# nexus1203/libBICOS

Measured on AMD Instinct MI355X. Metric: disparity Mpix/s + ms/match, 33x2 stack @ 2048x1536, 1/2/4/8 MI355X, higher is better.
Workload: dtype u8; 1 GPU; cfg2: 33x2 stack @ 2048x1536 u8, LIMITED 128-bit (4n-7=125 bits), nxcorr 0.96; n_images=33, rows=1536, cols=2048, descriptor_bits=128, rows_per_rank=1536, parallelism=single GPU

## Files before the change

### include/bicos_c.h

```cpp
#ifndef BICOS_C_H
#define BICOS_C_H

#include <stddef.h>
#include <stdint.h>

#ifdef __cplusplus
extern "C" {
#endif

#define BICOS_CV_8U 0
#define BICOS_CV_16U 2
#define BICOS_CV_16S 3
#define BICOS_CV_32F 5
#define BICOS_CV_64F 6

typedef struct {
    float nxcorr_threshold;
    float subpixel_step;
    float min_variance;
    int mode;
    int precision;
    int variant_type;
    int max_lr_diff;
    int no_dupes;
// ... 62 lines not shown
int bicos_match_host_range(bicos_engine* e, const void* const* stack0, const void* const* stack1,
                           int n, int rows, int cols, size_t step, int depth,
                           const BicosConfig* cfg, int has_nxcorr, int min_disparity,
                           int max_disparity, void* disparity, void* corrmap);


int bicos_match_host_multi(const int* devices, int ndev, const void* const* stack0,
                           const void* const* stack1, int n, int rows, int cols, size_t step,
                           int depth, const BicosConfig* cfg, int has_nxcorr, void* disparity,
                           void* corrmap);

int bicos_match_bands_device(const int* devices, int ndev, const void* const* stack0,
                             const void* const* stack1, const int* band_rows,
                             const size_t* row_pitch, const size_t* plane_pitch, int n, int cols,
                             int depth, const BicosConfig* cfg, int has_nxcorr, void* disparity,
                             void* corrmap);

size_t bicos_desc_pitch(int cols, int words);
int bicos_transform_device(const void* stack, int n, int rows, int cols, size_t row_pitch,
                           size_t plane_pitch, int depth, int mode, int words, uint32_t* desc,
                           void* stream);
int bicos_search_device(bicos_engine* e, const uint32_t* desc0, const uint32_t* desc1, int rows,
                        int cols, int words, int flags, int max_lr_diff, int16_t* out,
                        void* stream);
int bicos_search_device_range(bicos_engine* e, const uint32_t* desc0, const uint32_t* desc1,
                              int rows, int cols, int words, int flags, int max_lr_diff,
                              int min_disparity, int max_disparity, int16_t* out, void* stream);
int bicos_agree_device(const int16_t* raw, const void* stack0, const void* stack1, int n, int rows,
                       int cols, size_t row_pitch, size_t plane_pitch, int depth, float threshold,
                       int has_minvar, float minvar_scaled, float* out, float* corrmap,
                       void* stream);
int bicos_subpixel_device(const int16_t* raw, const void* stack0, const void* stack1, int n,
                          int rows, int cols, size_t row_pitch, size_t plane_pitch, int depth,
                          float threshold, float step, int has_minvar, float minvar_scaled,
                          float* out, float* corrmap, void* stream);
int bicos_agree_stage_device(const int16_t* raw, const void* stack0, const void* stack1, int n,
                             int rows, int cols, size_t row_pitch, size_t plane_pitch, int depth,
                             float threshold, float step, int has_minvar, float minvar_scaled,
                             int precision, float* out, void* corrmap, void* stream);

#define BICOS_PLAN_MATRIX_CORES 1
#define BICOS_PLAN_PACKED_KEYS 2
#define BICOS_PLAN_AGREE_IN_SEARCH 4
#define BICOS_PLAN_REVERSE_COMPACTED 8
#define BICOS_PLAN_CONSISTENCY_IN_AGREE 16
#define BICOS_PLAN_DENSE_ROWS 32
#define BICOS_PLAN_CONSISTENCY_ONE_PASS 64
int bicos_match_plan(bicos_engine* e, const void* stack0, const void* stack1, int n, int rows,
                     int cols, size_t row_pitch, size_t plane_pitch, int depth,
                     const BicosConfig* cfg, int has_nxcorr);
int bicos_search_packed(bicos_engine* e, int rows, int cols, int words, int bits, int n, int fused);
int bicos_agree_kernel(const void* stack0, const void* stack1, int n, size_t row_pitch,
                       size_t plane_pitch, int depth);

int bicos_search_agree_device(bicos_engine* e, const uint32_t* desc0, const uint32_t* desc1,
                              const void* stack0, const void* stack1, int n, int rows, int cols,
                              size_t row_pitch, size_t plane_pitch, int depth,
                              const BicosConfig* cfg, int has_nxcorr, void* disparity,
                              void* corrmap, void* stream);

#define BICOS_REPROJECT_ALLOW_NEGATIVE_Z 1
#define BICOS_REPROJECT_F32_SENTINEL 2
int bicos_reproject_device(bicos_engine* e, const void* disparity, int disp_type, int rows,
                           int cols, const double Q[16], int flags, float* xyz_map,
                           float* points, int32_t* index, size_t capacity, uint32_t* counts,
                           void* stream);
int bicos_reproject_host(bicos_engine* e, const void* disparity, int disp_type, int rows, int cols,
                         const double Q[16], int flags, float* xyz_map, float* points,
                         int32_t* index, size_t capacity, uint32_t counts[4]);
int bicos_reproject_segment(void);

#define BICOS_SPECKLE_F32_SENTINEL 1
int bicos_speckle_device(bicos_engine* e, const void* disparity, int disp_type, int rows, int cols,
                         int max_size, float max_diff, int flags, void* out, int32_t* labels,
                         uint32_t* counts, void* stream);
int bicos_speckle_host(bicos_engine* e, const void* disparity, int disp_type, int rows, int cols,
                       int max_size, float max_diff, int flags, void* out, int32_t* labels,
                       uint32_t counts[4]);
int bicos_speckle_tile(int* rows, int* cols);

int bicos_rectify_maps_device(const double K[9], const double* D, int nd, const double* R,
                              const double* P, int p_cols, int rows, int cols, float* map_x,
                              float* map_y, void* stream);
int bicos_rectify_maps_host(const double K[9], const double* D, int nd, const double* R,
                            const double* P, int p_cols, int rows, int cols, float* map_x,
                            float* map_y);
int bicos_rectify_device(bicos_engine* e, const void* src, int n, int src_rows, int src_cols,
                         size_t src_row_pitch, size_t src_plane_pitch, int depth,
                         const float* map_x, const float* map_y, size_t map_pitch, int rows,
                         int cols, void* dst, size_t dst_row_pitch, size_t dst_plane_pitch,
                         int border, uint8_t* valid, void* stream);
int bicos_rectify_host(bicos_engine* e, const void* const* src, int n, int src_rows, int src_cols,
                       size_t src_step, int depth, const float* map_x, const float* map_y,
                       size_t map_pitch, int rows, int cols, void* const* dst, size_t dst_step,
                       int border, uint8_t* valid);
int bicos_rectify_tile(int* rows, int* cols);

#define BICOS_MEDIAN_F32_SENTINEL 1
int bicos_median_device(bicos_engine* e, const void* disparity, int disp_type, int rows, int cols,
                        int ksize, int fill_min, int flags, void* out, uint32_t* counts, void* stream);
int bicos_median_host(bicos_engine* e, const void* disparity, int disp_type, int rows, int cols,
                      int ksize, int fill_min, int flags, void* out, uint32_t counts[4]);
int bicos_median_tile(int* rows, int* cols);

const char* bicos_build_info(void);

// ... 6 lines not shown
```

### libbicos_amd/_lib.py

```python
from __future__ import annotations

import ctypes
import os
import subprocess

_HERE = os.path.dirname(os.path.abspath(__file__))
LIB_PATH = os.path.join(_HERE, "libbicos_amd.so")
CSRC = os.path.join(_HERE, "csrc")

BICOS_OK = 0
BICOS_E_ARG = -1
BICOS_E_BITS = -2
BICOS_E_HIP = -3
BICOS_E_INTERNAL = -4

CV_8U, CV_16U, CV_16S, CV_32F, CV_64F = 0, 2, 3, 5, 6


class BicosConfig(ctypes.Structure):
    _fields_ = [
        ("nxcorr_threshold", ctypes.c_float),
        ("subpixel_step", ctypes.c_float),
        ("min_variance", ctypes.c_float),
        ("mode", ctypes.c_int),
        ("precision", ctypes.c_int),
        ("variant_type", ctypes.c_int),
        ("max_lr_diff", ctypes.c_int),
        ("no_dupes", ctypes.c_int),
    ]


class BicosResult(ctypes.Structure):
    _fields_ = [
        ("disparity_data", ctypes.c_void_p),
        ("disparity_rows", ctypes.c_int),
        ("disparity_cols", ctypes.c_int),
        ("disparity_type", ctypes.c_int),
        ("corrmap_data", ctypes.c_void_p),
        ("corrmap_rows", ctypes.c_int),
        ("corrmap_cols", ctypes.c_int),
        ("corrmap_type", ctypes.c_int),
    ]


EXPORTS = (
    "BICOS_CreateDefaultConfig", "BICOS_FreeConfig", "BICOS_FreeResult", "BICOS_Match",
    "BICOS_InvalidDisparityFloat", "BICOS_InvalidDisparityInt16", "bicos_last_error",
    "bicos_engine_create", "bicos_engine_default", "bicos_engine_destroy", "bicos_engine_tune", "bicos_descriptor_words", "bicos_output_type",
    "bicos_match_device", "bicos_match_device_i16", "bicos_match_host", "bicos_match_host_multi", "bicos_match_bands_device",
    "bicos_desc_pitch", "bicos_transform_device", "bicos_search_device",
    "bicos_agree_device", "bicos_subpixel_device", "bicos_agree_stage_device", "bicos_build_info",
    "bicos_match_plan", "bicos_search_agree_device", "bicos_search_packed", "bicos_agree_kernel",
    "bicos_match_device_range", "bicos_match_host_range", "bicos_search_device_range",
    "bicos_reproject_device", "bicos_reproject_host", "bicos_reproject_segment",
    "bicos_speckle_device", "bicos_speckle_host", "bicos_speckle_tile",
    "bicos_rectify_maps_device", "bicos_rectify_maps_host", "bicos_rectify_device",
    "bicos_rectify_host", "bicos_rectify_tile",
    "bicos_median_device", "bicos_median_host", "bicos_median_tile",
)

PLAN_MATRIX_CORES = 1
PLAN_PACKED_KEYS = 2
PLAN_AGREE_IN_SEARCH = 4
PLAN_REVERSE_COMPACTED = 8
PLAN_CONSISTENCY_IN_AGREE = 16
PLAN_DENSE_ROWS = 32
PLAN_CONSISTENCY_ONE_PASS = 64

REPROJECT_ALLOW_NEGATIVE_Z = 1
REPROJECT_F32_SENTINEL = 2

SPECKLE_F32_SENTINEL = 1

MEDIAN_F32_SENTINEL = 1


def build(verbose: bool = False, jobs: int = 4) -> str:
    out = subprocess.run(["make", "-C", CSRC, "-j%d" % jobs, "all"], capture_output=True,
                         text=True)
    if verbose:
        print(out.stdout, out.stderr)
    if out.returncode != 0:
        raise RuntimeError("libbicos_amd build failed:\n" + out.stdout[-4000:] + out.stderr[-4000:])
    return LIB_PATH


_lib = None


class BicosError(RuntimeError):
    pass


def lib() -> ctypes.CDLL:
    global _lib
    if _lib is not None:
        return _lib
    if not os.path.exists(LIB_PATH):
        raise ImportError("libbicos_amd.so not built at %s -- run libbicos_amd._lib.build() "
                          "(hipcc, gfx950)" % LIB_PATH)
    L = ctypes.CDLL(LIB_PATH)
    P, I, F, Z = ctypes.c_void_p, ctypes.c_int, ctypes.c_float, ctypes.c_size_t
    PI = ctypes.POINTER(ctypes.c_int)
    PP = ctypes.POINTER(ctypes.c_void_p)
    L.BICOS_CreateDefaultConfig.restype = ctypes.POINTER(BicosConfig)
# ... 4 lines not shown
    L.BICOS_FreeResult.restype = None
    L.BICOS_Match.argtypes = [PP, PI, PI, PI, I, PP, PI, PI, PI, I, ctypes.POINTER(BicosConfig)]
    L.BICOS_Match.restype = ctypes.POINTER(BicosResult)
    L.BICOS_InvalidDisparityFloat.restype = F
    L.BICOS_InvalidDisparityFloat.argtypes = []
    L.BICOS_InvalidDisparityInt16.restype = ctypes.c_int16
    L.BICOS_InvalidDisparityInt16.argtypes = []
    L.bicos_last_error.restype = ctypes.c_char_p
    L.bicos_last_error.argtypes = []
    L.bicos_engine_create.argtypes = [I, ctypes.POINTER(P)]
    L.bicos_engine_create.restype = I
    L.bicos_engine_default.argtypes = [I]
    L.bicos_engine_default.restype = P
    L.bicos_engine_destroy.argtypes = [P]
    L.bicos_engine_destroy.restype = None
    L.bicos_engine_tune.argtypes = [P, I, I, I, I]
    L.bicos_engine_tune.restype = I
    L.bicos_descriptor_words.argtypes = [I, I]
    L.bicos_descriptor_words.restype = I
    L.bicos_output_type.argtypes = [ctypes.POINTER(BicosConfig), I]
    L.bicos_output_type.restype = I
    L.bicos_match_device.argtypes = [P, P, P, I, I, I, Z, Z, I, ctypes.POINTER(BicosConfig), I,
                                     P, P, P]
    L.bicos_match_device.restype = I
    L.bicos_match_device_i16.argtypes = L.bicos_match_device.argtypes
    L.bicos_match_device_i16.restype = I
    L.bicos_match_host.argtypes = [P, PP, PP, I, I, I, Z, I, ctypes.POINTER(BicosConfig), I, P, P]
    L.bicos_match_host.restype = I
    PZ = ctypes.POINTER(ctypes.c_size_t)
    L.bicos_match_host_multi.argtypes = [PI, I, PP, PP, I, I, I, Z, I,
                                         ctypes.POINTER(BicosConfig), I, P, P]
    L.bicos_match_host_multi.restype = I
    L.bicos_match_bands_device.argtypes = [PI, I, PP, PP, PI, PZ, PZ, I, I, I,
                                           ctypes.POINTER(BicosConfig), I, P, P]
    L.bicos_match_bands_device.restype = I
    L.bicos_desc_pitch.argtypes = [I, I]
    L.bicos_desc_pitch.restype = Z
    L.bicos_transform_device.argtypes = [P, I, I, I, Z, Z, I, I, I, P, P]
    L.bicos_transform_device.restype = I
    L.bicos_search_device.argtypes = [P, P, P, I, I, I, I, I, P, P]
    L.bicos_search_device.restype = I
    L.bicos_agree_device.argtypes = [P, P, P, I, I, I, Z, Z, I, F, I, F, P, P, P]
    L.bicos_agree_device.restype = I
    L.bicos_subpixel_device.argtypes = [P, P, P, I, I, I, Z, Z, I, F, F, I, F, P, P, P]
    L.bicos_subpixel_device.restype = I
    L.bicos_agree_stage_device.argtypes = [P, P, P, I, I, I, Z, Z, I, F, F, I, F, I, P, P, P]
    L.bicos_agree_stage_device.restype = I
    L.bicos_match_plan.argtypes = [P, P, P, I, I, I, Z, Z, I, ctypes.POINTER(BicosConfig), I]
    L.bicos_match_plan.restype = I
    L.bicos_search_packed.argtypes = [P, I, I, I, I, I, I]
    L.bicos_search_packed.restype = I
    L.bicos_agree_kernel.argtypes = [P, P, I, Z, Z, I]
    L.bicos_agree_kernel.restype = I
    L.bicos_search_agree_device.argtypes = [P, P, P, P, P, I, I, I, Z, Z, I,
                                            ctypes.POINTER(BicosConfig), I, P, P, P]
    L.bicos_search_agree_device.restype = I
    L.bicos_match_device_range.argtypes = [P, P, P, I, I, I, Z, Z, I, ctypes.POINTER(BicosConfig),
                                           I, I, I, P, P, P]
    L.bicos_match_device_range.restype = I
    L.bicos_match_host_range.argtypes = [P, PP, PP, I, I, I, Z, I, ctypes.POINTER(BicosConfig), I,
                                         I, I, P, P]
    L.bicos_match_host_range.restype = I
    L.bicos_search_device_range.argtypes = [P, P, P, I, I, I, I, I, I, I, P, P]
    L.bicos_search_device_range.restype = I
    PD = ctypes.POINTER(ctypes.c_double)
    L.bicos_reproject_device.argtypes = [P, P, I, I, I, PD, I, P, P, P, Z, P, P]
    L.bicos_reproject_device.restype = I
    L.bicos_reproject_host.argtypes = [P, P, I, I, I, PD, I, P, P, P, Z, P]
    L.bicos_reproject_host.restype = I
    L.bicos_reproject_segment.argtypes = []
    L.bicos_reproject_segment.restype = I
    L.bicos_speckle_device.argtypes = [P, P, I, I, I, I, F, I, P, P, P, P]
    L.bicos_speckle_device.restype = I
    L.bicos_speckle_host.argtypes = [P, P, I, I, I, I, F, I, P, P, P]
    L.bicos_speckle_host.restype = I
    L.bicos_speckle_tile.argtypes = [PI, PI]
    L.bicos_speckle_tile.restype = I
    L.bicos_rectify_maps_device.argtypes = [PD, PD, I, PD, PD, I, I, I, P, P, P]
    L.bicos_rectify_maps_device.restype = I
    L.bicos_rectify_maps_host.argtypes = [PD, PD, I, PD, PD, I, I, I, P, P]
    L.bicos_rectify_maps_host.restype = I
    L.bicos_rectify_device.argtypes = [P, P, I, I, I, Z, Z, I, P, P, Z, I, I, P, Z, Z, I, P, P]
    L.bicos_rectify_device.restype = I
    L.bicos_rectify_host.argtypes = [P, PP, I, I, I, Z, I, P, P, Z, I, I, PP, Z, I, P]
    L.bicos_rectify_host.restype = I
    L.bicos_rectify_tile.argtypes = [PI, PI]
    L.bicos_rectify_tile.restype = I
    L.bicos_median_device.argtypes = [P, P, I, I, I, I, I, I, P, P, P]
    L.bicos_median_device.restype = I
    L.bicos_median_host.argtypes = [P, P, I, I, I, I, I, I, P, P]
    L.bicos_median_host.restype = I
    L.bicos_median_tile.argtypes = [PI, PI]
    L.bicos_median_tile.restype = I
    L.bicos_build_info.restype = ctypes.c_char_p
    L.bicos_build_info.argtypes = []
    _lib = L
    return L


def check_disparity_range(rng):
    if rng is None:
        return None
    try:
        lo, hi = rng
    except (TypeError, ValueError):
        raise ValueError("disparity_range must be None or a pair (lo, hi)") from None
# ... 96 lines not shown
```

### libbicos_amd/csrc/entries.cpp

```cpp
#include "engine.hpp"
#include "reproject.hpp"
#include "speckle.hpp"
#include "median.hpp"

#include <cmath>
#include <vector>

using namespace bicos_impl;

namespace {

int check_words(int words) {
    if (words == 1 || words == 2 || words == 4 || words == 8) return BICOS_OK;
    return fail(BICOS_E_ARG, "words must be 1, 2, 4 or 8");
}

int match_device_entry(bicos_engine* e, const void* stack0, const void* stack1, int n, int rows,
                       int cols, size_t row_pitch, size_t plane_pitch, int depth,
                       const BicosConfig* cfg, int has_nxcorr, void* disparity, void* corrmap,
                       void* stream, bool disp_i16, const DispRange* range = nullptr,
                       const uint32_t* desc0 = nullptr, const uint32_t* desc1 = nullptr) {
    if (range)
        if (int rc0 = check_range(range->min, range->max)) return rc0;
    if (!cfg) return fail(BICOS_E_ARG, "null config");
// ... 175 lines not shown
}

int bicos_match_device(bicos_engine* e, const void* stack0, const void* stack1, int n, int rows,
                       int cols, size_t row_pitch, size_t plane_pitch, int depth,
                       const BicosConfig* cfg, int has_nxcorr, void* disparity, void* corrmap,
                       void* stream) {
    return match_device_entry(e, stack0, stack1, n, rows, cols, row_pitch, plane_pitch, depth, cfg,
                              has_nxcorr, disparity, corrmap, stream, false);
}

int bicos_match_device_range(bicos_engine* e, const void* stack0, const void* stack1, int n,
                             int rows, int cols, size_t row_pitch, size_t plane_pitch, int depth,
                             const BicosConfig* cfg, int has_nxcorr, int min_disparity,
                             int max_disparity, void* disparity, void* corrmap, void* stream) {
    const DispRange range{min_disparity, max_disparity};
    return match_device_entry(e, stack0, stack1, n, rows, cols, row_pitch, plane_pitch, depth, cfg,
                              has_nxcorr, disparity, corrmap, stream, false, &range);
}

int bicos_match_device_i16(bicos_engine* e, const void* stack0, const void* stack1, int n, int rows,
                           int cols, size_t row_pitch, size_t plane_pitch, int depth,
                           const BicosConfig* cfg, int has_nxcorr, void* disparity, void* corrmap,
                           void* stream) {
    return match_device_entry(e, stack0, stack1, n, rows, cols, row_pitch, plane_pitch, depth, cfg,
                              has_nxcorr, disparity, corrmap, stream, true);
}

int bicos_match_plan(bicos_engine* e, const void* stack0, const void* stack1, int n, int rows,
                     int cols, size_t row_pitch, size_t plane_pitch, int depth,
                     const BicosConfig* cfg, int has_nxcorr) {
    if (!cfg) return fail(BICOS_E_ARG, "null config");
    if (int rc0 = check_stack_shape(n, depth, 0, 0)) return rc0;
    if (descriptor_words(n, cfg->mode ? 1 : 0) < 0) return fail(BICOS_E_BITS, "input stacks too large");
    return match_plan(e, n, rows, cols, row_pitch, plane_pitch, depth, *cfg, has_nxcorr != 0,
                      stack0, stack1).bits();
}

int bicos_search_packed(bicos_engine* e, int rows, int cols, int words, int bits, int n, int fused) {
    return search_runs_packed(e, rows, cols, words, bits, n, fused != 0) ? 1 : 0;
}

int bicos_agree_kernel(const void* stack0, const void* stack1, int n, size_t row_pitch,
                       size_t plane_pitch, int depth) {
    if (int rc0 = check_stack_shape(n, depth, 0, 0)) return rc0;
    bicos_hip::AgreeArgs aa{};
    aa.stack0 = stack0;
    aa.stack1 = stack1;
    aa.n = n;
    aa.row_pitch = row_pitch;
    aa.plane_pitch = plane_pitch;
    return bicos_hip::agree_kernel_kind(aa, depth);
}

int bicos_search_agree_device(bicos_engine* e, const uint32_t* desc0, const uint32_t* desc1,
                              const void* stack0, const void* stack1, int n, int rows, int cols,
                              size_t row_pitch, size_t plane_pitch, int depth,
                              const BicosConfig* cfg, int has_nxcorr, void* disparity,
                              void* corrmap, void* stream) {
    if (!cfg) return fail(BICOS_E_ARG, "null config");
    if (!e) return fail(BICOS_E_ARG, "null engine");
    if (rows > 0 && cols > 0 && (!desc0 || !desc1)) return fail(BICOS_E_ARG, "null descriptors");
    return match_device_entry(e, stack0, stack1, n, rows, cols, row_pitch, plane_pitch, depth, cfg,
                              has_nxcorr, disparity, corrmap, stream, false, nullptr, desc0, desc1);
}

int bicos_match_host(bicos_engine* e, const void* const* stack0, const void* const* stack1, int n,
                     int rows, int cols, size_t step, int depth, const BicosConfig* cfg,
                     int has_nxcorr, void* disparity, void* corrmap) {
    return match_host_entry(e, stack0, stack1, n, rows, cols, step, depth, cfg, has_nxcorr,
                            disparity, corrmap, nullptr);
}

int bicos_match_host_range(bicos_engine* e, const void* const* stack0, const void* const* stack1,
                           int n, int rows, int cols, size_t step, int depth,
                           const BicosConfig* cfg, int has_nxcorr, int min_disparity,
                           int max_disparity, void* disparity, void* corrmap) {
    const DispRange range{min_disparity, max_disparity};
    return match_host_entry(e, stack0, stack1, n, rows, cols, step, depth, cfg, has_nxcorr,
                            disparity, corrmap, &range);
}

int bicos_transform_device(const void* stack, int n, int rows, int cols, size_t row_pitch,
                           size_t plane_pitch, int depth, int mode, int words, uint32_t* desc,
                           void* stream) {
    if (int rc0 = check_stack_shape(n, depth, 0, 0)) return rc0;
    if (int rc0 = check_words(words)) return rc0;
    const int need = descriptor_words(n, mode ? 1 : 0);
    if (need < 0 || need > words) return fail(BICOS_E_BITS, "descriptor too narrow for n");
    uint32_t span = 0;
    if (int rc0 = stack_span(n, rows, cols, row_pitch, plane_pitch, depth, &span)) return rc0;
    bicos_hip::TransformArgs ta{stack, nullptr, desc, nullptr, n, rows, cols,
                                row_pitch, plane_pitch, bicos_desc_pitch(cols, words), 0, span};
    return check_hip(bicos_hip::launch_transform(ta, depth, mode ? 1 : 0, words, (hipStream_t)stream),
                     "transform launch");
}

int bicos_search_device(bicos_engine* e, const uint32_t* desc0, const uint32_t* desc1, int rows,
                        int cols, int words, int flags, int max_lr_diff, int16_t* out,
                        void* stream) {
    return search_entry(e, desc0, desc1, rows, cols, words, flags, max_lr_diff, nullptr, out,
                        stream);
}

int bicos_search_device_range(bicos_engine* e, const uint32_t* desc0, const uint32_t* desc1,
                              int rows, int cols, int words, int flags, int max_lr_diff,
                              int min_disparity, int max_disparity, int16_t* out, void* stream) {
// ... 221 lines not shown
```

### libbicos_amd/csrc/kernels.hip

```cpp
#include "kernels.hpp"
#include "nxc.hpp"
#include "stack.hpp"
#include "transform.hpp"

#include <hip/hip_runtime.h>
#include <stdint.h>

#include <algorithm>
#include <cstdlib>
#include <cstring>

#include <type_traits>

namespace bicos_hip {

namespace {

constexpr int16_t INVALID_I16 = -32768;

__device__ __forceinline__ float fdiv_rn(float a, float b) { return __fdiv_rn(a, b); }

__device__ __forceinline__ uint32_t bcnt_acc(uint32_t x, uint32_t acc) {
    asm("" : "+v"(acc));
    return __builtin_popcount(x) + acc;
}


using nxc::ld;
using nxc::fma_p;
using nxc::div_p;
using nxc::sqrt_p;
using nxc::nxcorr_dev;



template <int WORDS>
struct BitWriter {
    uint32_t w[WORDS];
    uint32_t cur = 0;
    int nbits = 0;
    int widx = 0;

    __device__ __forceinline__ BitWriter() {
#pragma unroll
        for (int k = 0; k < WORDS; ++k) w[k] = 0;
    }
    __device__ __forceinline__ void flush() {
#pragma unroll
        for (int k = 0; k < WORDS; ++k)
            if (k == widx) w[k] = cur;
    }
    __device__ __forceinline__ void set(bool v) {
        cur |= (uint32_t)v << nbits;
        if (++nbits == 32) {
            flush();
            ++widx;
// ... 55 lines not shown
                bw.set((float)a0 < av);
                ps[t] = a0 + b0;
                a0 = b0;
                b0 = c0;
            }
        }
#pragma unroll
        for (int t = 0; t < 15; ++t)
            if (t == n - 2) ps[t] = a0 + b0;
        bw.set(a0 < b0);
        bw.set((float)a0 < av);
        bw.set((float)b0 < av);
#pragma unroll
        for (int t = 0; t < 15; ++t)
#pragma unroll
            for (int i = 0; i < 15; ++i)
                if (t < n - 1 && i < n - 1 && i != t && i != t - 1 && i != t + 1)
                    bw.set(ps[t] < ps[i]);
    }
    bw.finish();

    if (WORDS % 4 == 0) {
#pragma unroll
        for (int k = 0; k < WORDS; k += 4)
            *(uint4*)(out + k) = make_uint4(bw.w[k], bw.w[k + 1], bw.w[k + 2], bw.w[k + 3]);
    } else if (WORDS == 2) {
        *(uint2*)out = make_uint2(bw.w[0], bw.w[1 % WORDS]);
    } else {
        out[0] = bw.w[0];
    }
}

template <typename TIn, int WORDS, int MAXN, bool EXACT>
__global__ __launch_bounds__(256) void transform_limited_kernel(TransformArgs a) {
    const int col = blockIdx.x * 256 + threadIdx.x;
    const int row = blockIdx.y;
    const int which = blockIdx.z;
    if (col >= a.cols) return;
    const StackReader<TIn> rd(which ? a.stack1 : a.stack0, a.stack_bytes);
    uint32_t* __restrict__ out = (which ? a.desc1 : a.desc0) + (size_t)row * a.desc_pitch + (size_t)col * WORDS;
    const uint32_t pp = (uint32_t)a.plane_pitch;
    const uint32_t rowoff = (uint32_t)row * (uint32_t)a.row_pitch;
    uint32_t w[WORDS];
    limited_descriptor<TIn, WORDS, MAXN, EXACT>(rd, (uint32_t)col, rowoff, pp, a.n, a.magic, w);

    if (WORDS % 4 == 0) {
#pragma unroll
        for (int k = 0; k < WORDS; k += 4)
            *(uint4*)(out + k) = make_uint4(w[k], w[k + 1], w[k + 2], w[k + 3]);
    } else if (WORDS == 2) {
        *(uint2*)out = make_uint2(w[0], w[1 % WORDS]);
    } else {
        out[0] = w[0];
    }
}

template <typename TIn, int WORDS, int N>
__global__ __launch_bounds__(256) void transform_full_kernel(TransformArgs a) {
    const int col = blockIdx.x * 256 + threadIdx.x;
    const int row = blockIdx.y;
    const int which = blockIdx.z;
    if (col >= a.cols) return;
    const StackReader<TIn> rd(which ? a.stack1 : a.stack0, a.stack_bytes);
    uint32_t* __restrict__ out = (which ? a.desc1 : a.desc0) + (size_t)row * a.desc_pitch + (size_t)col * WORDS;
    uint32_t w[WORDS];
    full_descriptor<TIn, WORDS, N>(rd, (uint32_t)col, (uint32_t)row * (uint32_t)a.row_pitch,
                                   (uint32_t)a.plane_pitch, a.magic, w);
    if (WORDS % 4 == 0) {
#pragma unroll
        for (int k = 0; k < WORDS; k += 4)
            *(uint4*)(out + k) = make_uint4(w[k], w[k + 1], w[k + 2], w[k + 3]);
    } else if (WORDS == 2) {
        *(uint2*)out = make_uint2(w[0], w[1 % WORDS]);
    } else {
        out[0] = w[0];
    }
}


template <int WORDS>
__device__ __forceinline__ uint32_t ham(const uint32_t (&a)[WORDS], const uint32_t (&b)[WORDS]) {
    uint32_t c = __builtin_popcount(a[0] ^ b[0]);
#pragma unroll
    for (int k = 1; k < WORDS; ++k) c = bcnt_acc(a[k] ^ b[k], c);
    return c;
}

template <int WORDS>
__device__ __forceinline__ void lds_fetch(const uint32_t* s, uint32_t (&d)[WORDS]) {
    if (WORDS >= 4) {
#pragma unroll
        for (int k = 0; k < WORDS; k += 4) {
            const uint4 v = *(const uint4*)(s + k);
            d[k] = v.x;
            d[(k + 1) % WORDS] = v.y;
            d[(k + 2) % WORDS] = v.z;
            d[(k + 3) % WORDS] = v.w;
        }
    } else if (WORDS == 2) {
        const uint2 v = *(const uint2*)s;
        d[0] = v.x;
        d[1 % WORDS] = v.y;
    } else {
        d[0] = s[0];
    }
}
// ... 307 lines not shown
    uint32_t r[MAXN];
#pragma unroll
    for (int t = 0; t < MAXN; ++t)
        r[t] = rd1(c1, rowoff + (uint32_t)min(t, n - 1) * pp);
#pragma unroll
    for (int j = 0; j < PASSES; ++j) {
        const int p = j * WPP + p0;
        if (p < n) tile_l[p * DW + threadIdx.x % DW] = w[j];
    }
    __syncthreads();
    if (!live) return;
    const TIn* lt = (const TIn*)tile_l + threadIdx.x;
    const size_t o = (size_t)row * a.cols + col;
    TPrec corr = (TPrec)__builtin_nan("");
    if (inb) {
        uint32_t sl = 0, sr = 0;
#pragma unroll
        for (int t = 0; t < MAXN; ++t)
            if (t < n) {
                sl += lt[t * 256];
                sr += r[t];
                if ((t & 7) == 7) __builtin_amdgcn_sched_barrier(0);
            }
        asm volatile("" ::: "memory");
        const TPrec m0 = div_p((TPrec)sl, (TPrec)n);
        const TPrec m1 = div_p((TPrec)sr, (TPrec)n);
        TPrec cov = 0, v0 = 0, v1 = 0;
#pragma unroll
        for (int t = 0; t < MAXN; ++t)
            if (t < n) {
                const TPrec x0 = (TPrec)(uint32_t)lt[t * 256] - m0;
                const TPrec x1 = (TPrec)r[t] - m1;
                cov = fma_p(x0, x1, cov);
                v0 = fma_p(x0, x0, v0);
                v1 = fma_p(x1, x1, v1);
                if ((t & 7) == 7) __builtin_amdgcn_sched_barrier(0);
            }
        if (a.has_minvar && (v0 < (TPrec)a.minvar || v1 < (TPrec)a.minvar))
            corr = (TPrec)-1;
        else
            corr = div_p(cov, sqrt_p(v0 * v1));
        if (corr < (TPrec)a.threshold) d = INVALID_I16;
    } else {
        d = INVALID_I16;
    }
    if (a.out_f32)
        ((float*)a.out)[o] = (float)d;
    else
        ((int16_t*)a.out)[o] = (int16_t)d;
    if (a.corrmap) ((TPrec*)a.corrmap)[o] = corr;
}


template <typename TIn, int WORDS, int MAXN>
hipError_t launch_tl(const TransformArgs& a, dim3 grid, hipStream_t st) {
    if (a.n == MAXN)
        hipLaunchKernelGGL((transform_limited_kernel<TIn, WORDS, MAXN, true>), grid, dim3(256), 0, st, a);
    else
        hipLaunchKernelGGL((transform_limited_kernel<TIn, WORDS, MAXN, false>), grid, dim3(256), 0, st, a);
    return hipGetLastError();
}

template <typename TIn, int WORDS>
hipError_t launch_transform_w(const TransformArgs& a, int mode, hipStream_t st) {
    dim3 grid((a.cols + 255) / 256, a.rows, a.stack1 ? 2 : 1);
    if (mode == 0) {
        const int n = a.n;
        if constexpr (WORDS == 1) return launch_tl<TIn, WORDS, 9>(a, grid, st);
        else if constexpr (WORDS == 2) return n <= 12 ? launch_tl<TIn, WORDS, 12>(a, grid, st)
                                                      : launch_tl<TIn, WORDS, 17>(a, grid, st);
        else if constexpr (WORDS == 4) return n <= 24 ? launch_tl<TIn, WORDS, 24>(a, grid, st)
                                                      : launch_tl<TIn, WORDS, 33>(a, grid, st);
        else if (n <= 40) return launch_tl<TIn, WORDS, 40>(a, grid, st);
        else if (n <= 48) return launch_tl<TIn, WORDS, 48>(a, grid, st);
        else return launch_tl<TIn, WORDS, 65>(a, grid, st);
    }
#define BICOS_FULL_N(N)                                                                   \
    case N:                                                                               \
        if constexpr (WORDS == (N * N - 2 * N + 3 <= 32 ? 1 : N * N - 2 * N + 3 <= 64 ? 2  \
                                : N * N - 2 * N + 3 <= 128 ? 4 : 8)) {                     \
            hipLaunchKernelGGL((transform_full_kernel<TIn, WORDS, N>), grid, dim3(256), 0, st, a); \
            return hipGetLastError();                                                     \
        }                                                                                 \
        break;
    switch (a.n) {
        BICOS_FULL_N(2) BICOS_FULL_N(3) BICOS_FULL_N(4) BICOS_FULL_N(5) BICOS_FULL_N(6)
        BICOS_FULL_N(7) BICOS_FULL_N(8) BICOS_FULL_N(9) BICOS_FULL_N(10) BICOS_FULL_N(11)
        BICOS_FULL_N(12) BICOS_FULL_N(13) BICOS_FULL_N(14) BICOS_FULL_N(15) BICOS_FULL_N(16)
    }
#undef BICOS_FULL_N
    hipLaunchKernelGGL((transform_kernel<TIn, WORDS, 1>), grid, dim3(256), 0, st, a);
    return hipGetLastError();
}

template <typename TIn>
hipError_t launch_transform_t(const TransformArgs& a, int mode, int words, hipStream_t st) {
    switch (words) {
        case 1: return launch_transform_w<TIn, 1>(a, mode, st);
        case 2: return launch_transform_w<TIn, 2>(a, mode, st);
        case 4: return launch_transform_w<TIn, 4>(a, mode, st);
        case 8: return launch_transform_w<TIn, 8>(a, mode, st);
    }
    return hipErrorInvalidValue;
}

template <int WORDS, bool NODUPES, int RP>
hipError_t launch_search16_r(const SearchArgs& a, int waves, hipStream_t st) {
    const size_t stage = (size_t)a.chunk * WORDS * 4;
// ... 80 lines not shown
    g.variant = 16;
    const int max_chunk = max_lds_bytes / (words * 4 + extra_col_bytes);
    g.chunk = cols < max_chunk ? cols : max_chunk;
    g.waves = waves ? waves : 8;
    g.R = R == 4 ? 4 : 2;
    if (split) {
        g.split = split;
    } else {
        const long base = (long)rows * ((cols + 64L * g.R - 1) / (64L * g.R));
        const int tiles256 = (cols + 255) / 256;
        const double slots = (double)(cus > 0 ? cus : 256) * 32.0;
        double best = -1.0;
        g.split = 1;
        for (int sp = 1; sp <= 8; sp *= 2) {
            if (sp > 1 && (tiles256 < sp || g.waves % sp)) break;
            const double rounds = (double)(base * sp) / slots;
            const double fill = rounds / __builtin_ceil(rounds);
            const double score = fill + 0.1 * (rounds < 3.0 ? rounds : 3.0) / 3.0 -
                                 0.005 * (double)__builtin_ctz(sp);
            if (score > best + 1e-9) {
                best = score;
                g.split = sp;
            }
        }
    }
    const long per_wg = 64L * (g.waves / g.split) * g.R;
    g.tiles_per_row = (int)((cols + per_wg - 1) / per_wg);
    return g;
}

hipError_t launch_search(SearchArgs a, const SearchGeometry& g, int words, bool nodupes,
                         hipStream_t st) {
    if (a.rows <= 0 || a.cols <= 0) return hipSuccess;
    a.chunk = g.chunk;
    a.tiles_per_row = g.tiles_per_row;
    a.split = g.split;
    if (g.waves % g.split) return hipErrorInvalidValue;
    switch (words) {
        case 1: return launch_search_w<1>(a, nodupes, g, st);
        case 2: return launch_search_w<2>(a, nodupes, g, st);
        case 4: return launch_search_w<4>(a, nodupes, g, st);
        case 8: return launch_search_w<8>(a, nodupes, g, st);
    }
    return hipErrorInvalidValue;
}

hipError_t launch_consistency(const ConsistencyArgs& a, hipStream_t st) {
    if (a.rows <= 0 || a.cols <= 0) return hipSuccess;
    dim3 grid((a.cols + 255) / 256, a.rows);
    hipLaunchKernelGGL(consistency_kernel, grid, dim3(256), 0, st, a);
    return hipGetLastError();
}

int agree_kernel_kind(const AgreeArgs& a, int depth) {
    if (a.n > 65) return 0;
    return agree_dwords_aligned(a, depth == 1 ? 1 : 2) ? 2 : 1;
}

hipError_t launch_agree(const AgreeArgs& a, int depth, bool dbl, hipStream_t st) {
    if (a.rows <= 0 || a.cols <= 0) return hipSuccess;
    if (depth == 1)
        return dbl ? launch_agree_t<uint8_t, double>(a, st) : launch_agree_t<uint8_t, float>(a, st);
    return dbl ? launch_agree_t<uint16_t, double>(a, st) : launch_agree_t<uint16_t, float>(a, st);
}

}
```

### libbicos_amd/csrc/kernels.hpp

```cpp
#pragma once

#include <hip/hip_runtime.h>
#include <stddef.h>
#include <stdint.h>

namespace bicos_hip {

struct TransformArgs {
    const void* stack0;
    const void* stack1;
    uint32_t* desc0;
    uint32_t* desc1;
    int n, rows, cols;
    size_t row_pitch;
    size_t plane_pitch;
    size_t desc_pitch;
    uint32_t magic;
    uint32_t stack_bytes;
};

struct AgreeArgs {
    const int16_t* raw;
    size_t raw_pitch;
    const void* stack0;
// ... 13 lines not shown
    const int16_t* rev;
    int max_lr_diff;
};

struct SearchArgs {
    const uint32_t* desc0;
    const uint32_t* desc1;
    int16_t* out;
    int rows, cols;
    size_t desc_pitch;
    size_t out_pitch;
    int out_mode;
    int chunk;
    int tiles_per_row;
    int split;
    int tail_col0;
    int tail_T;
    const int16_t* keep;
    size_t keep_pitch;
    uint8_t* row_valid;
    size_t valid_pitch;
};

struct SearchAgreeArgs {
    SearchArgs s;
    AgreeArgs ag;
};

struct SearchRangeArgs {
    SearchArgs s;
    int dmin, dmax;
};

struct SearchGeometry {
    int chunk;
    int waves;
    int R;
    int tiles_per_row;
    int variant;
    int split;
};

struct ConsistencyArgs {
    const int16_t* fwd;
    const int16_t* rev;
    int16_t* out;
    int rows, cols;
    size_t out_pitch;
    int max_lr_diff;
};


hipError_t launch_transform(TransformArgs a, int depth, int mode, int words, hipStream_t st);
SearchGeometry search_geometry(int rows, int cols, int words, int max_lds_bytes, int variant = 16,
                               int R = 0, int waves = 0, int split = 0, int cus = 256,
                               int extra_col_bytes = 0);
hipError_t launch_search(SearchArgs a, const SearchGeometry& g, int words, bool nodupes,
                         hipStream_t st);
hipError_t launch_consistency(const ConsistencyArgs& a, hipStream_t st);

struct MxGeometry {
    int chunk;
    int waves;
    int T;
    int tiles_per_row;
    int keys;
    int ksteps;
    int fk;
    int tail_T;
    int tail_col0;
    int pk;
    int pk_T;
    int pk_chunk;
    int pk_tiles_per_row;
    int pk_tail_col0;
    int stream;
    int prune;
    int packed;
};
MxGeometry search_mx_geometry(int rows, int cols, int words, int lds_bytes, int T = 0,
                              int waves = 0, int cus = 256, int keys = 0, int bits = 0);
hipError_t launch_search_mx(SearchArgs a, const MxGeometry& g, int words, bool nodupes,
                            hipStream_t st);
bool search_mx_agree_fusable(const MxGeometry& g, int words, bool nodupes, int cols, int n,
                             int depth, bool dbl);
hipError_t launch_search_mx_agree(SearchArgs a, const AgreeArgs& ag, const MxGeometry& g, int words,
                                  hipStream_t st);
bool search_mx_packed(const MxGeometry& g, int rows, int cols, int words, int n);
bool search_lr_eligible(int words, int bits, int cols);
hipError_t launch_search_lr(SearchArgs a, int words, int bits, int max_lr_diff, hipStream_t st);
hipError_t launch_search_range(SearchArgs a, int dmin, int dmax, int words, bool nodupes,
                               int bits, int cus, hipStream_t st, int tiles = 0,
                               int waves_wg = 0);
hipError_t launch_agree(const AgreeArgs& a, int depth, bool dbl, hipStream_t st);
int agree_kernel_kind(const AgreeArgs& a, int depth);
hipError_t launch_subpixel(const AgreeArgs& a, int depth, bool dbl, hipStream_t st);
hipError_t launch_subpixel_wide(const AgreeArgs& a, int depth, bool dbl, hipStream_t st);

}
```

### libbicos_amd/device.py

```python
from __future__ import annotations

import ctypes
import dataclasses
from typing import Optional, Sequence, Tuple

import torch

from . import _lib

INVALID_I16 = -32768


@dataclasses.dataclass
class MatchConfig:
    nxcorr_threshold: Optional[float] = 0.5
    subpixel_step: Optional[float] = None
    min_variance: Optional[float] = None
    mode: int = 0
    precision: int = 0
    variant: int = 0
    max_lr_diff: int = 1
    no_dupes: bool = False
    disparity_range: Optional[Tuple[int, int]] = None

# ... 98 lines not shown
        corr_dtype = torch.float64 if cfg.precision else torch.float32
        i16 = (out is not None and has_nxcorr and out.dtype == torch.int16 and
               cfg.subpixel_step is None)
        if i16:
            disp_dtype = torch.int16
        if out is None:
            out = torch.empty((rows, cols), dtype=disp_dtype, device=dev)
        _check_out(out, "out", (rows, cols), (disp_dtype,), dev)
        if has_nxcorr and want_corrmap and corrmap is None:
            corrmap = torch.empty((rows, cols), device=dev, dtype=corr_dtype)
        if not (has_nxcorr and want_corrmap):
            corrmap = None
        if corrmap is not None:
            _check_out(corrmap, "corrmap", (rows, cols), (corr_dtype,), dev)
        rng = _lib.check_disparity_range(cfg.disparity_range)
        if rng is not None and i16:
            raise ValueError("disparity_range is not supported with an int16 `out` map")
        if rng is not None:
            rc = self._L.bicos_match_device_range(
                self._h, stack0.data_ptr(), stack1.data_ptr(), n, rows, cols, rp, pp,
                _depth(stack0), ctypes.byref(c), has_nxcorr, rng[0], rng[1], out.data_ptr(),
                corrmap.data_ptr() if corrmap is not None else None, _stream(dev, stream))
            _lib.check(rc, "bicos_match_device_range")
            return out, corrmap
        entry = self._L.bicos_match_device_i16 if i16 else self._L.bicos_match_device
        rc = entry(
            self._h, stack0.data_ptr(), stack1.data_ptr(), n, rows, cols, rp, pp, _depth(stack0),
            ctypes.byref(c), has_nxcorr, out.data_ptr(),
            corrmap.data_ptr() if corrmap is not None else None, _stream(dev, stream))
        _lib.check(rc, "bicos_match_device")
        return out, corrmap

    def plan(self, stack0: torch.Tensor, stack1: torch.Tensor,
             cfg: Optional[MatchConfig] = None) -> int:
        cfg = cfg or MatchConfig()
        n, rows, cols, rp, pp = _check_stack(stack0)
        c, has_nxcorr = cfg.to_c()
        rc = self._L.bicos_match_plan(self._h, stack0.data_ptr(), stack1.data_ptr(), n, rows, cols,
                                      rp, pp, _depth(stack0), ctypes.byref(c), has_nxcorr)
        if rc < 0:
            _lib.check(rc, "bicos_match_plan")
        return rc

    def search_packed(self, rows: int, cols: int, words: int = 4, bits: int = 0, n: int = 0,
                      fused: bool = False) -> bool:
        return bool(self._L.bicos_search_packed(self._h, rows, cols, words, bits, n, int(fused)))

    def agree_kernel(self, stack0: torch.Tensor, stack1: torch.Tensor) -> int:
        n, rows, cols, rp, pp = _check_stack(stack0)
        rc = self._L.bicos_agree_kernel(stack0.data_ptr(), stack1.data_ptr(), n, rp, pp,
                                        _depth(stack0))
        if rc < 0:
            _lib.check(rc, "bicos_agree_kernel")
        return rc

    def search_agree(self, desc0: torch.Tensor, desc1: torch.Tensor, stack0: torch.Tensor,
                     stack1: torch.Tensor, cfg: Optional[MatchConfig] = None,
                     out: Optional[torch.Tensor] = None, corrmap: Optional[torch.Tensor] = None,
                     stream=None) -> Tuple[torch.Tensor, Optional[torch.Tensor]]:
        cfg = cfg or MatchConfig()
        n, rows, cols, rp, pp = _check_stack(stack0)
        if tuple(stack1.shape) != (n, rows, cols) or stack1.stride() != stack0.stride() or \
                stack1.dtype != stack0.dtype:
            raise ValueError("stack1 must match stack0 in shape, strides and dtype")
        words = descriptor_words(n, cfg.mode)
        pitch = self._L.bicos_desc_pitch(cols, words)
        for name, d in (("desc0", desc0), ("desc1", desc1)):
            if d.device != stack0.device or d.dtype != torch.int32 or not d.is_contiguous() or \
                    tuple(d.shape) != (rows, pitch):
                raise ValueError("%s must be a contiguous int32 [%d, %d] tensor on %s"
                                 % (name, rows, pitch, stack0.device))
        c, has_nxcorr = cfg.to_c()
        dev = stack0.device
        disp_dtype = torch.float32 if has_nxcorr else torch.int16
        corr_dtype = torch.float64 if cfg.precision else torch.float32
        if out is None:
            out = torch.empty((rows, cols), dtype=disp_dtype, device=dev)
        _check_out(out, "out", (rows, cols), (disp_dtype,), dev)
        if has_nxcorr and corrmap is None:
            corrmap = torch.empty((rows, cols), device=dev, dtype=corr_dtype)
        if not has_nxcorr:
            corrmap = None
        if corrmap is not None:
            _check_out(corrmap, "corrmap", (rows, cols), (corr_dtype,), dev)
        rc = self._L.bicos_search_agree_device(
            self._h, desc0.data_ptr(), desc1.data_ptr(), stack0.data_ptr(), stack1.data_ptr(),
            n, rows, cols, rp, pp, _depth(stack0), ctypes.byref(c), has_nxcorr, out.data_ptr(),
            corrmap.data_ptr() if corrmap is not None else None, _stream(dev, stream))
        _lib.check(rc, "bicos_search_agree_device")
        return out, corrmap

    def _reproject_args(self, disp: torch.Tensor, Q):
        if not disp.is_cuda:
            raise ValueError("device API needs CUDA/HIP tensors")
        if disp.dim() != 2:
            raise ValueError("disparity map must be [rows, cols]")
        if disp.dtype not in (torch.int16, torch.float32):
            raise ValueError("disparity map must be int16 or float32, got %s" % disp.dtype)
        if not disp.is_contiguous():
            raise ValueError("disparity map must be contiguous (dense rows)")
        rows, cols = disp.shape
        if rows * cols >= 2 ** 31:
            raise ValueError("disparity map has more than 2^31 - 1 pixels")
        typ = _lib.CV_32F if disp.dtype == torch.float32 else _lib.CV_16S
        return rows, cols, typ, _lib.reproject_q(Q)

# ... 317 lines not shown
```

Measured before the change: 10190 Mpix/s.

## Add packed SWAR limited-transform kernel computing two pixels per 32-bit lane

New measurement: 10410 Mpix/s (median of 6 runs). 2.2% higher.

```diff
diff --git a/include/bicos_c.h b/include/bicos_c.h
--- a/include/bicos_c.h
+++ b/include/bicos_c.h
@@ -138,6 +138,8 @@
 int bicos_search_packed(bicos_engine* e, int rows, int cols, int words, int bits, int n, int fused);
 int bicos_agree_kernel(const void* stack0, const void* stack1, int n, size_t row_pitch,
                        size_t plane_pitch, int depth);
+int bicos_transform_kernel(const void* stack0, const void* stack1, int n, int rows, int cols,
+                           size_t row_pitch, size_t plane_pitch, int depth, int mode, int words);
 
 int bicos_search_agree_device(bicos_engine* e, const uint32_t* desc0, const uint32_t* desc1,
                               const void* stack0, const void* stack1, int n, int rows, int cols,
diff --git a/libbicos_amd/_lib.py b/libbicos_amd/_lib.py
--- a/libbicos_amd/_lib.py
+++ b/libbicos_amd/_lib.py
@@ -51,6 +51,7 @@
     "bicos_desc_pitch", "bicos_transform_device", "bicos_search_device",
     "bicos_agree_device", "bicos_subpixel_device", "bicos_agree_stage_device", "bicos_build_info",
     "bicos_match_plan", "bicos_search_agree_device", "bicos_search_packed", "bicos_agree_kernel",
+    "bicos_transform_kernel",
     "bicos_match_device_range", "bicos_match_host_range", "bicos_search_device_range",
     "bicos_reproject_device", "bicos_reproject_host", "bicos_reproject_segment",
     "bicos_speckle_device", "bicos_speckle_host", "bicos_speckle_tile",
@@ -161,6 +162,8 @@
     L.bicos_search_packed.restype = I
     L.bicos_agree_kernel.argtypes = [P, P, I, Z, Z, I]
     L.bicos_agree_kernel.restype = I
+    L.bicos_transform_kernel.argtypes = [P, P, I, I, I, Z, Z, I, I, I]
+    L.bicos_transform_kernel.restype = I
     L.bicos_search_agree_device.argtypes = [P, P, P, P, P, I, I, I, Z, Z, I,
                                             ctypes.POINTER(BicosConfig), I, P, P, P]
     L.bicos_search_agree_device.restype = I
diff --git a/libbicos_amd/csrc/entries.cpp b/libbicos_amd/csrc/entries.cpp
--- a/libbicos_amd/csrc/entries.cpp
+++ b/libbicos_amd/csrc/entries.cpp
@@ -251,6 +251,24 @@
     return bicos_hip::agree_kernel_kind(aa, depth);
 }
 
+int bicos_transform_kernel(const void* stack0, const void* stack1, int n, int rows, int cols,
+                           size_t row_pitch, size_t plane_pitch, int depth, int mode, int words) {
+    if (int rc0 = check_stack_shape(n, depth, 0, 0)) return rc0;
+    if (int rc0 = check_words(words)) return rc0;
+    uint32_t span = 0;
+    if (int rc0 = stack_span(n, rows, cols, row_pitch, plane_pitch, depth, &span)) return rc0;
+    bicos_hip::TransformArgs ta{};
+    ta.stack0 = stack0;
+    ta.stack1 = stack1;
+    ta.n = n;
+    ta.rows = rows;
+    ta.cols = cols;
+    ta.row_pitch = row_pitch;
+    ta.plane_pitch = plane_pitch;
+    ta.stack_bytes = span;
+    return bicos_hip::transform_kernel_kind(ta, depth, mode ? 1 : 0, words);
+}
+
 int bicos_search_agree_device(bicos_engine* e, const uint32_t* desc0, const uint32_t* desc1,
                               const void* stack0, const void* stack1, int n, int rows, int cols,
                               size_t row_pitch, size_t plane_pitch, int depth,
diff --git a/libbicos_amd/csrc/kernels.hip b/libbicos_amd/csrc/kernels.hip
--- a/libbicos_amd/csrc/kernels.hip
+++ b/libbicos_amd/csrc/kernels.hip
@@ -2,6 +2,7 @@
 #include "nxc.hpp"
 #include "stack.hpp"
 #include "transform.hpp"
+#include "transform_pk.hpp"
 
 #include <hip/hip_runtime.h>
 #include <stdint.h>
@@ -163,6 +164,83 @@
         *(uint2*)out = make_uint2(w[0], w[1 % WORDS]);
     } else {
         out[0] = w[0];
+    }
+}
+
+template <int WORDS, int N>
+__global__ __launch_bounds__(256) void transform_limited_pk_kernel(TransformArgs a) {
+    constexpr int PX = 4;
+    const uint32_t lane = threadIdx.x & 63u;
+    const uint32_t col = (blockIdx.x * 256 + threadIdx.x) * PX;
+    const uint32_t wave_col = col - lane * PX;
+    const uint32_t cols = (uint32_t)a.cols;
+    const int row = blockIdx.y;
+    const int which = blockIdx.z;
+    if (wave_col >= cols) return;
+    const __amdgpu_buffer_rsrc_t r = __builtin_amdgcn_make_buffer_rsrc(
+        const_cast<void*>(which ? a.stack1 : a.stack0), (short)0, (int)((a.stack_bytes + 3u) & ~3u),
+        0x00020000);
+    const uint32_t pp = (uint32_t)a.plane_pitch;
+    const uint32_t rowoff = (uint32_t)row * (uint32_t)a.row_pitch;
+
+    uint32_t d[N];
+#pragma unroll
+    for (int t = 0; t < N; ++t)
+        d[t] = __builtin_amdgcn_raw_buffer_load_b32(r, col, rowoff + (uint32_t)t * pp, 0);
+    const auto even = [&](int t) { return tpk::even_pixels(d[t]); };
+    const auto odd = [&](int t) { return tpk::odd_pixels(d[t]); };
+    const uint32_t thr_e = tpk::pair_threshold(tpk::pair_sum<N>(even), N, a.magic);
+    const uint32_t thr_o = tpk::pair_threshold(tpk::pair_sum<N>(odd), N, a.magic);
+#pragma unroll
+    for (int t = 0; t < N; ++t) asm volatile("" : "+v"(d[t]));
+    uint32_t acc_e[tpk::accumulators(N)], acc_o[tpk::accumulators(N)];
+    tpk::pair_bits<N>(even, thr_e, acc_e);
+    tpk::pair_bits<N>(odd, thr_o, acc_o);
+    uint32_t w0[WORDS], w1[WORDS], w2[WORDS], w3[WORDS];
+    tpk::pair_words<WORDS>(acc_e, w0, w2);
+    tpk::pair_words<WORDS>(acc_o, w1, w3);
+    uint32_t w[PX * WORDS];
+#pragma unroll
+    for (int k = 0; k < WORDS; ++k) {
+        w[k] = w0[k];
+        w[WORDS + k] = w1[k];
+        w[2 * WORDS + k] = w2[k];
+        w[3 * WORDS + k] = w3[k];
+    }
+
+    uint32_t* __restrict__ orow = (which ? a.desc1 : a.desc0) + (size_t)row * a.desc_pitch;
+    constexpr int LW = PX * WORDS;
+    if constexpr (LW == 4) {
+        uint32_t* __restrict__ out = orow + col;
+        if (col + PX <= cols) {
+            *(uint4*)out = make_uint4(w[0], w[1], w[2], w[3]);
+        } else {
+#pragma unroll
+            for (int i = 0; i < PX - 1; ++i)
+                if (col + i < cols) out[i] = w[i];
+        }
+    } else {
+        typedef uint32_t u32x4 __attribute__((ext_vector_type(4)));
+        typedef uint32_t u32x2 __attribute__((ext_vector_type(2)));
+        __shared__ __attribute__((aligned(16))) uint32_t stage[256 * LW];
+        uint32_t* sw = stage + (threadIdx.x - lane) * LW;
+#pragma unroll
+        for (int k = 0; k < LW; k += 4)
+            *(uint4*)(sw + lane * LW + k) = make_uint4(w[k], w[k + 1], w[k + 2], w[k + 3]);
+        __builtin_amdgcn_fence(__ATOMIC_RELEASE, "wavefront");
+        __builtin_amdgcn_wave_barrier();
+        __builtin_amdgcn_fence(__ATOMIC_ACQUIRE, "wavefront");
+        const uint32_t wave_cols = cols - wave_col < 64u * PX ? cols - wave_col : 64u * PX;
+        const uint32_t valid = wave_cols * WORDS;
+        uint32_t* __restrict__ out = orow + (size_t)wave_col * WORDS;
+#pragma unroll
+        for (int k = 0; k < LW / 4; ++k) {
+            const uint32_t q = (k * 64 + lane) * 4;
+            if (q + 4 <= valid)
+                __builtin_nontemporal_store(*(const u32x4*)(sw + q), (u32x4*)(out + q));
+            else if (WORDS == 2 && q + 2 <= valid)
+                __builtin_nontemporal_store(*(const u32x2*)(sw + q), (u32x2*)(out + q));
+        }
     }
 }
 
@@ -576,8 +654,32 @@
 }
 
 
+bool transform_pk_enabled() {
+    static const bool on = [] {
+        const char* v = std::getenv("BICOS_TRANSFORM_PK");
+        return !(v && v[0] == '0' && v[1] == 0);
+    }();
+    return on;
+}
+
+constexpr uint64_t PK_CACHED_STACK_BYTES = 256ull << 20;
+
+bool transform_pk_eligible(const TransformArgs& a, int depth, int mode, int words) {
+    return transform_pk_enabled() && depth == 1 && mode == 0 && tpk::built(a.n) &&
+           words == tpk::limited_words(a.n) && (uintptr_t)a.stack0 % 4 == 0 &&
+           (uintptr_t)a.stack1 % 4 == 0 && a.row_pitch % 4 == 0 && a.plane_pitch % 4 == 0 &&
+           (uint64_t)a.stack_bytes * (a.stack1 ? 2 : 1) <= PK_CACHED_STACK_BYTES;
+}
+
 template <typename TIn, int WORDS, int MAXN>
 hipError_t launch_tl(const TransformArgs& a, dim3 grid, hipStream_t st) {
+    if constexpr (sizeof(TIn) == 1 && tpk::built(MAXN) && WORDS == tpk::limited_words(MAXN)) {
+        if (transform_pk_eligible(a, 1, 0, WORDS)) {
+            const dim3 grid4((a.cols + 1023) / 1024, grid.y, grid.z);
+            hipLaunchKernelGGL((transform_limited_pk_kernel<WORDS, MAXN>), grid4, dim3(256), 0, st, a);
+            return hipGetLastError();
+        }
+    }
     if (a.n == MAXN)
         hipLaunchKernelGGL((transform_limited_kernel<TIn, WORDS, MAXN, true>), grid, dim3(256), 0, st, a);
     else
@@ -764,6 +866,10 @@
     return hipGetLastError();
 }
 
+int transform_kernel_kind(const TransformArgs& a, int depth, int mode, int words) {
+    return transform_pk_eligible(a, depth, mode, words) ? 1 : 0;
+}
+
 int agree_kernel_kind(const AgreeArgs& a, int depth) {
     if (a.n > 65) return 0;
     return agree_dwords_aligned(a, depth == 1 ? 1 : 2) ? 2 : 1;
diff --git a/libbicos_amd/csrc/kernels.hpp b/libbicos_amd/csrc/kernels.hpp
--- a/libbicos_amd/csrc/kernels.hpp
+++ b/libbicos_amd/csrc/kernels.hpp
@@ -89,6 +89,7 @@
 
 
 hipError_t launch_transform(TransformArgs a, int depth, int mode, int words, hipStream_t st);
+int transform_kernel_kind(const TransformArgs& a, int depth, int mode, int words);
 SearchGeometry search_geometry(int rows, int cols, int words, int max_lds_bytes, int variant = 16,
                                int R = 0, int waves = 0, int split = 0, int cus = 256,
                                int extra_col_bytes = 0);
diff --git a/libbicos_amd/csrc/transform_pk.hpp b/libbicos_amd/csrc/transform_pk.hpp
--- /dev/null
+++ b/libbicos_amd/csrc/transform_pk.hpp
@@ -0,0 +1,116 @@
+#pragma once
+
+#include <stdint.h>
+
+#if defined(__HIP__)
+#define BICOS_TPK_FN __host__ __device__ inline
+#else
+#define BICOS_TPK_FN inline
+#endif
+#if defined(__HIP_DEVICE_COMPILE__)
+#define BICOS_TPK_STEP_DONE() __builtin_amdgcn_sched_barrier(0)
+#define BICOS_TPK_KEEP(x) asm("" : "+v"(x))
+#else
+#define BICOS_TPK_STEP_DONE() ((void)0)
+#define BICOS_TPK_KEEP(x) ((void)0)
+#endif
+
+namespace bicos_hip {
+namespace tpk {
+
+constexpr uint32_t BIAS = 0x7FFF7FFFu;
+constexpr uint32_t SIGN = 0x80008000u;
+
+constexpr int loop_bits(int n) { return n >= 4 ? 6 + 4 * (n - 4) : 3 * (n - 2); }
+constexpr int limited_bits(int n) { return loop_bits(n) + 4; }
+constexpr int accumulators(int n) { return (limited_bits(n) + 15) / 16; }
+constexpr int limited_words(int n) {
+    return n < 2 ? 0 : limited_bits(n) <= 32 ? 1 : limited_bits(n) <= 64 ? 2
+         : limited_bits(n) <= 128 ? 4 : limited_bits(n) <= 256 ? 8 : 0;
+}
+constexpr bool built(int n) {
+    return n == 9 || n == 12 || n == 17 || n == 24 || n == 33 || n == 40 || n == 48 || n == 65;
+}
+
+BICOS_TPK_FN uint32_t left(uint32_t X) { return BIAS - X; }
+BICOS_TPK_FN uint32_t less(uint32_t nx, uint32_t Y) { return nx + Y; }
+
+template <int K, int ACC>
+BICOS_TPK_FN void put(uint32_t (&acc)[ACC], uint32_t nx, uint32_t Y) {
+    static_assert(K >= 0 && K / 16 < ACC, "bit outside the accumulators");
+    const uint32_t d = less(nx, Y) & SIGN;
+    acc[K / 16] |= d >> (15 - K % 16);
+    BICOS_TPK_KEEP(acc[K / 16]);
+}
+
+BICOS_TPK_FN uint32_t ceil_div(uint32_t sum, uint32_t n, uint32_t magic) {
+    return (uint32_t)(((uint64_t)(sum + n - 1) * magic) >> 32);
+}
+
+template <int N, class Sample>
+BICOS_TPK_FN uint32_t pair_sum(const Sample& X) {
+    uint32_t sum = 0;
+#pragma unroll
+    for (int t = 0; t < N; ++t) sum += X(t);
+    return sum;
+}
+BICOS_TPK_FN uint32_t pair_threshold(uint32_t sum, uint32_t n, uint32_t magic) {
+    return ceil_div(sum & 0xFFFFu, n, magic) | ceil_div(sum >> 16, n, magic) << 16;
+}
+
+template <int T, int N, int ACC, class Sample>
+BICOS_TPK_FN void steps(const Sample& X, uint32_t a, uint32_t b, uint32_t ps2, uint32_t ps1,
+                        uint32_t thr, uint32_t (&acc)[ACC]) {
+    const uint32_t na = left(a);
+    const uint32_t cur = a + b;
+    if constexpr (T < N - 2) {
+        constexpr int pos = T < 2 ? 3 * T : 6 + 4 * (T - 2);
+        const uint32_t c = X(T + 2);
+        put<pos>(acc, na, b);
+        put<pos + 1>(acc, na, c);
+        put<pos + 2>(acc, na, thr);
+        if constexpr (T >= 2) put<pos + 3>(acc, left(ps2), cur);
+        BICOS_TPK_STEP_DONE();
+        steps<T + 1, N, ACC>(X, b, c, ps1, cur, thr, acc);
+    } else {
+        constexpr int nl = loop_bits(N);
+        put<nl>(acc, na, b);
+        put<nl + 1>(acc, na, thr);
+        put<nl + 2>(acc, left(b), thr);
+        if constexpr (N >= 4)
+            put<nl + 3>(acc, left(ps2), cur);
+        else
+            acc[(nl + 3) / 16] |= 0x00010001u << ((nl + 3) % 16);
+    }
+}
+
+template <int N, class Sample>
+BICOS_TPK_FN void pair_bits(const Sample& X, uint32_t thr, uint32_t (&acc)[accumulators(N)]) {
+    static_assert(N >= 2 && N <= 65, "fields hold sums of at most 65 u8 samples");
+#pragma unroll
+    for (int j = 0; j < accumulators(N); ++j) acc[j] = 0;
+    steps<0, N, accumulators(N)>(X, X(0), X(1), 0u, 0u, thr, acc);
+}
+
+template <int N, class Sample>
+BICOS_TPK_FN void pair_descriptor(const Sample& X, uint32_t magic, uint32_t (&acc)[accumulators(N)]) {
+    pair_bits<N>(X, pair_threshold(pair_sum<N>(X), N, magic), acc);
+}
+
+template <int WORDS, int ACC>
+BICOS_TPK_FN void pair_words(const uint32_t (&acc)[ACC], uint32_t (&lo)[WORDS], uint32_t (&hi)[WORDS]) {
+    static_assert(ACC <= 2 * WORDS, "descriptor too narrow");
+#pragma unroll
+    for (int m = 0; m < WORDS; ++m) {
+        const uint32_t a = 2 * m < ACC ? acc[2 * m] : 0u;
+        const uint32_t b = 2 * m + 1 < ACC ? acc[2 * m + 1] : 0u;
+        lo[m] = (a & 0xFFFFu) | b << 16;
+        hi[m] = a >> 16 | (b & 0xFFFF0000u);
+    }
+}
+
+BICOS_TPK_FN uint32_t even_pixels(uint32_t dword) { return dword & 0x00FF00FFu; }
+BICOS_TPK_FN uint32_t odd_pixels(uint32_t dword) { return dword >> 8 & 0x00FF00FFu; }
+
+}
+}
diff --git a/libbicos_amd/device.py b/libbicos_amd/device.py
--- a/libbicos_amd/device.py
+++ b/libbicos_amd/device.py
@@ -174,6 +174,17 @@
                                         _depth(stack0))
         if rc < 0:
             _lib.check(rc, "bicos_agree_kernel")
+        return rc
+
+    def transform_kernel(self, stack0: torch.Tensor, stack1: Optional[torch.Tensor] = None,
+                         mode: int = 0, words: Optional[int] = None) -> int:
+        n, rows, cols, rp, pp = _check_stack(stack0)
+        words = words or descriptor_words(n, mode)
+        rc = self._L.bicos_transform_kernel(
+            stack0.data_ptr(), stack1.data_ptr() if stack1 is not None else None, n, rows, cols,
+            rp, pp, _depth(stack0), mode, words)
+        if rc < 0:
+            _lib.check(rc, "bicos_transform_kernel")
         return rc
 
     def search_agree(self, desc0: torch.Tensor, desc1: torch.Tensor, stack0: torch.Tensor,
```
